# luigifreda/plvs

Hardware: AMD Instinct MI355X
Metric: Mvoxels/sec TSDF integrate (chisel 5 cm / 5 m, 640x480 RGB-D) (higher is better)
Workload: dtype f32; 1 GPU; configs[2] stand-in, STREAMING: see DESIGN.md 4.1 / 4.6; mode=order-free (fixed-point sums; sdf / weight within tolerance), longest_voxel_run=25008, parallelism=chunk-hash shard x1

## Files before the change

### plvs_amd/csrc/tsdf_walk.hpp

```cpp
#pragma once
#include <hip/hip_runtime.h>

#include <cstdint>

#include "tsdf_chisel_core.hpp"
#include "tsdf_directory.hpp"
#include "tsdf_tiles.hpp"
#include "tsdf_walk_table.hpp"

namespace {

using namespace plvs::chisel;
using plvs::tsdf::cloud_of;
using plvs::tsdf::tile_span;
using plvs::tsdf::tile_span_tables;
using plvs::tsdf::TileSpan;
using plvs::tsdf::kCoordBias;
using plvs::tsdf::kErrCoordRange;
using plvs::tsdf::kErrDirectoryMiss;
using plvs::tsdf::kErrPoolFull;
using plvs::tsdf::home_bucket;
using plvs::tsdf::next_bucket;

constexpr int kWalkRays = 512;
constexpr int kMaskWords = kWalkRays / 32;
#ifndef PLVS_WALK_ENTRIES
#define PLVS_WALK_ENTRIES 4096
#endif
constexpr int kWalkEntries = PLVS_WALK_ENTRIES;
constexpr int kWalkLimit = kWalkEntries * 7 / 8;
constexpr int kWalkWindow = kWalkLimit / 2;
constexpr int kWalkChunks = 64;
constexpr uint32_t kErrScratch = 8u;

#ifdef PLVS_WALK_PROF
__device__ unsigned long long g_walk_prof[16];
__device__ unsigned long long g_apply_items[8192][4];
#define WALK_PROF_BEGIN()                                         \
  long long prof_t = (long long)clock64();                        \
  unsigned long long prof_acc[9] = {0, 0, 0, 0, 0, 0, 0, 0, 0}
#define WALK_PROF(k)                                               \
  do {                                                             \
    const long long now = (long long)clock64();                    \
    prof_acc[k] += (unsigned long long)(now - prof_t);             \
    prof_t = now;                                                  \
  } while (0)
#define WALK_PROF_END()                                            \
  do {                                                             \
    if (threadIdx.x == 0)                                          \
      for (int k = 0; k < 9; ++k) atomicAdd(&g_walk_prof[k], prof_acc[k]); \
  } while (0)
#else
#define WALK_PROF_BEGIN() do {} while (0)
#define WALK_PROF(k) do {} while (0)
#define WALK_PROF_END() do {} while (0)
#endif

struct WalkCounters {
  unsigned long long total_visits;
  uint32_t err;
  uint32_t num_heads;
  uint32_t num_updated;
  uint32_t max_run;
  uint32_t num_desc;
  uint32_t run_need;
  uint32_t rec_top, seg_top;
  uint32_t ncold;
  uint32_t split_tiles;
  uint32_t num_parts;
  uint32_t num_multi;
  uint32_t ndeferred;
  uint32_t ndeferred2;
  uint32_t over_small;
  uint32_t skip;
  uint32_t collect_top;
  uint32_t collect_parts;
  uint32_t ndeferred3;
};

constexpr int kLogLen = 16;
constexpr int kSlabs = 8;
constexpr int kSlabVox = kChunkVox / kSlabs;

struct SubTile {
  uint16_t lo, hi;
  uint32_t vlo, vhi;
  int32_t cloud;
};

constexpr uint32_t kKeyEmpty = 0xFFFFFFFFu;
constexpr int kBuckets = kWalkEntries / 4;
constexpr int kOriginBias = 512;

constexpr int log2_of(int v) { return v <= 1 ? 0 : 1 + log2_of(v / 2); }
struct WalkShared {
  static constexpr int kEntries = kWalkEntries, kBucketCount = kWalkEntries / 4, kLogLen = ::kLogLen;
  alignas(16) uint32_t ekey[kWalkEntries];
  int32_t org[3];
  uint32_t cand[kWalkRays / 64];
  int32_t worg[kWalkRays / 64][3];
  uint32_t run_total, vis_total;
  uint32_t ccode[kWalkChunks];
  int32_t cslot[kWalkChunks];
  uint32_t ccnt[kWalkChunks * kSlabs];
  uint16_t cbase[kWalkChunks * kSlabs];
  uint32_t rbase;
  SubTile stack[16];
  int sp;
  uint32_t nent;
  uint32_t overflow;
  uint32_t wsum[kWalkRays / 64];
  uint32_t next, nrays;
};
template <int E>
struct FastShared {
  static constexpr int kEntries = E, kBucketCount = E / 4, kLogLen = E == 1536 ? ::kLogLen - 1 : ::kLogLen;
  static_assert(E % kWalkRays == 0 && E >= 1024, "every thread owns E / kWalkRays entries (and a bucket four)");
  alignas(16) uint32_t ekey[E];
  uint32_t cand[kWalkRays / 64];
  int32_t worg[kWalkRays / 64][3];
  uint32_t run_total, vis_total;
  uint32_t ccode[kWalkChunks];
  int32_t cslot[kWalkChunks];
  uint32_t ccnt[kWalkChunks * kSlabs];
  uint16_t cbase[kWalkChunks * kSlabs];
  uint32_t rcnt[kWalkChunks * kSlabs];
  uint16_t rcbase[kWalkChunks * kSlabs];
  uint32_t any_cold;
  uint32_t nent, overflow;
};


__device__ __forceinline__ bool rel_key(int vx, int vy, int vz, int ox, int oy, int oz, uint32_t* key) {
  const uint32_t dx = (uint32_t)(vx - ox), dy = (uint32_t)(vy - oy), dz = (uint32_t)(vz - oz);
  *key = dx | (dy << 10) | (dz << 20);
  return ((dx | dy | dz) >> 10) == 0u;
}
__device__ __forceinline__ int origin_of(int v) { return (v - kOriginBias) & ~15; }
constexpr uint32_t kChunkCodeMask = 0x3F0FC3F0u;
__device__ __forceinline__ uint32_t chunk_code(uint32_t key) { return key & kChunkCodeMask; }
__device__ __forceinline__ uint32_t voxel_in_chunk(uint32_t key) {
  return (key & 15u) | ((key >> 6) & 0xF0u) | ((key >> 12) & 0xF00u);
}
__device__ __forceinline__ void chunk_of_code(uint32_t code, int ox, int oy, int oz, int* cx, int* cy, int* cz) {
  *cx = (ox >> 4) + (int)((code >> 4) & 63u);
  *cy = (oy >> 4) + (int)((code >> 14) & 63u);
  *cz = (oz >> 4) + (int)((code >> 24) & 63u);
}
constexpr uint32_t kKeyMul = plvs::tsdf::kTableKeyMul, kKeyMulInv = plvs::tsdf::kTableKeyMulInv;
__device__ __forceinline__ uint32_t table_key(uint32_t key) { return key * kKeyMul; }
__device__ __forceinline__ uint32_t voxel_key(uint32_t tkey) { return tkey * kKeyMulInv; }
template <class SH>
__device__ __forceinline__ uint32_t key_bucket(uint32_t tkey) { return home_bucket<SH::kBucketCount>(tkey); }

__device__ __forceinline__ uint32_t wave_scan_incl(uint32_t x) {
  x += (uint32_t)__builtin_amdgcn_update_dpp(0, (int)x, 0x111, 0xf, 0xf, false);
  x += (uint32_t)__builtin_amdgcn_update_dpp(0, (int)x, 0x112, 0xf, 0xf, false);
  x += (uint32_t)__builtin_amdgcn_update_dpp(0, (int)x, 0x114, 0xf, 0xf, false);
  x += (uint32_t)__builtin_amdgcn_update_dpp(0, (int)x, 0x118, 0xf, 0xf, false);
  x += (uint32_t)__builtin_amdgcn_update_dpp(0, (int)x, 0x142, 0xa, 0xf, false);
// ... 669 lines not shown
      if (!own_region) {
        __syncthreads();
        rbase = S.rbase;
      }
#pragma unroll
      for (int k = 0; k < kPer; ++k) {
        if (slot_of[k] < 0) continue;
        const int e = tid + k * kWalkRays;
        const uint32_t vid = vkey[k] % (uint32_t)kChunkVox;
        const uint4 r = make_uint4(vid | ((uint32_t)(ewc[k] >> 32) << 12),
                                   grid ? grid_order_key(*grid, gt, elast[k]) : first + elast[k], (uint32_t)e_wuu[e],
                                   (uint32_t)ewc[k]);
        uint32_t at;
        if (ci[k] >= 0) {
          at = rbase + S.cbase[ci[k] * kSlabs + (int)(vid / kSlabVox)] + rank[k];
        } else {
          at = ntiles * rec_stride + atomicAdd(&ctr->rec_top, 1u);
          const uint32_t sg = ntiles * (uint32_t)kWalkChunks + atomicAdd(&ctr->seg_top, 1u);
          if (at >= out.rec_cap || sg >= out.seg_cap) {
            atomicOr(&ctr->err, kErrScratch);
          } else {
            uint32_t sub[kSlabs];
#pragma unroll
            for (int s = 0; s < kSlabs; ++s) sub[s] = (uint32_t)s > vid / kSlabVox ? 1u : 0u;
            out.seg[2 * (size_t)sg] = make_uint4((uint32_t)slot_of[k], at, 1u, gtile);
            out.seg[2 * (size_t)sg + 1] = pack_suboffsets(sub);
            if (out.chunk_nseg) atomicAdd(&out.chunk_nseg[slot_of[k]], 1u);
          }
        }
        if (at < out.rec_cap) out.rec[at] = r;
      }
    }

    ++flushes;
    WALK_PROF(6);
    if (!kRuns) {
      if (single && !was_split) break;
      continue;
    }
    uint32_t inc = nneed;
#pragma unroll
    for (int off = 1; off < 64; off <<= 1) {
      const uint32_t up = (uint32_t)__shfl_up((int)inc, off);
      if (lane >= off) inc += up;
    }
    const uint32_t wave_runs = (uint32_t)__shfl((int)inc, 63);
    if (!any_multi) {
      uint32_t base = 0;
      if (lane == 0 && wave_runs) base = atomicAdd(&S.run_total, wave_runs);
      base = (uint32_t)__shfl((int)base, 0);
      const bool fits_runs = base + wave_runs <= (1u << runs.r1_log2);
      if (!fits_runs && lane == 0) {
        atomicOr(&ctr->err, kErrScratch);
        atomicMax(&ctr->run_need, base + wave_runs);
      }
      uint32_t m = base + inc - nneed;
#pragma unroll
      for (int k = 0; k < kPer; ++k) {
        if (!(need & (1u << k)) || !fits_runs) continue;
        const size_t d = ((size_t)tile << runs.r1_log2) + m++;
        runs.dkey[d] = vkey[k];
        uint4* dst = reinterpret_cast<uint4*>(runs.masks + d * kMaskWords);
        const uint32_t word = elast[k] >> 5, bit = 1u << (elast[k] & 31u);
#pragma unroll
        for (int q = 0; q < kMaskWords / 4; ++q)
          dst[q] = make_uint4(word == 4u * q ? bit : 0u, word == 4u * q + 1u ? bit : 0u, word == 4u * q + 2u ? bit : 0u,
                              word == 4u * q + 3u ? bit : 0u);
      }
      WALK_PROF(7);
      if (single && !was_split) break;
      continue;
    }
    if (lane == 63) S.wsum[wid] = inc;
    __syncthreads();
    uint32_t wbase = 0, nruns = 0;
#pragma unroll
    for (int w = 0; w < kWalkRays / 64; ++w) {
      const uint32_t v = S.wsum[w];
      if (w < wid) wbase += v;
      nruns += v;
    }
    const uint32_t emitted = S.run_total;
    const bool fits_runs = emitted + nruns <= (1u << runs.r1_log2);
    if (!fits_runs && tid == 0) {
      atomicOr(&ctr->err, kErrScratch);
      atomicMax(&ctr->run_need, emitted + nruns);
    }
    {
      uint32_t m = wbase + inc - nneed;
#pragma unroll
      for (int k = 0; k < kPer; ++k) e_midx[tid + k * kWalkRays] = (need & (1u << k)) ? (uint16_t)m++ : (uint16_t)0xFFFFu;
    }
    for (uint32_t r0 = 0; fits_runs && r0 < nruns; r0 += kMaskCap) {
      __syncthreads();
#pragma unroll
      for (int k = 0; k < kMaskCap * kMaskWords / kWalkRays; ++k) raw[tid + k * kWalkRays] = 0u;
      __syncthreads();
      if (walks && nmine) {
        const uint32_t logged = min(nmine, (uint32_t)kLogLen);
        for (uint32_t k = 0; k < logged; ++k) {
          const uint32_t m = (uint32_t)e_midx[vlog[k * kWalkRays + tid]] - r0;
          if (m < (uint32_t)kMaskCap) atomicOr(&raw[m * kMaskWords + (tid >> 5)], 1u << (tid & 31));
        }
        if (nmine > (uint32_t)kLogLen) {
          walk_one(P, pose, ray, st.vlo, st.vhi, [&](uint32_t k, int vx, int vy, int vz, float) {
            if (k >= (uint32_t)kLogLen) {
              uint32_t key;
              const int e = rel_key(vx, vy, vz, fox, foy, foz, &key) ? table_find(S, table_key(key)) : -1;
              const uint32_t m = e >= 0 ? (uint32_t)e_midx[e] - r0 : 0xFFFFFFFFu;
              if (m < (uint32_t)kMaskCap) atomicOr(&raw[m * kMaskWords + (tid >> 5)], 1u << (tid & 31));
            }
            return true;
          });
        }
      }
      __syncthreads();
#pragma unroll
      for (int k = 0; k < kPer; ++k) {
        const uint32_t m = (uint32_t)e_midx[tid + k * kWalkRays];
        if (m == 0xFFFFu || m < r0 || m >= r0 + (uint32_t)kMaskCap) continue;
        const size_t d = ((size_t)tile << runs.r1_log2) + emitted + m;
        runs.dkey[d] = vkey[k];
        const uint32_t* mk = raw + (m - r0) * kMaskWords;
        uint4* dst = reinterpret_cast<uint4*>(runs.masks + d * kMaskWords);
#pragma unroll
        for (int q = 0; q < kMaskWords / 4; ++q) dst[q] = make_uint4(mk[4 * q], mk[4 * q + 1], mk[4 * q + 2], mk[4 * q + 3]);
      }
    }
    __syncthreads();
    if (tid == 0) S.run_total = emitted + nruns;
    WALK_PROF(7);
    if (single && !was_split) break;
  }

#pragma unroll
  for (int off = 32; off > 0; off >>= 1) my_visits += (uint32_t)__shfl_xor((int)my_visits, off);
  if (lane == 0 && my_visits) atomicAdd(&S.vis_total, my_visits);
  __syncthreads();
  if (tid == 0) {
    if (kRuns) runs.run_cnt[tile] = min(S.run_total, 1u << runs.r1_log2);
    if (kAcc) {
      out.tile_visits[tile] = S.vis_total;
      if (flushes == 0) out.seg_cnt[tile] = 0;
    }
    if (was_split) atomicAdd(&ctr->split_tiles, 1u);
  }
  WALK_PROF(8);
  WALK_PROF_END();
  }
}

constexpr int walk_fast_waves(int E) { return E > 2048 ? 2 : (E > 1536 ? 4 : 6); }
constexpr int kFastEntriesSmall = 1536;
template <int E, bool kGrid>
__device__ __forceinline__ void walk_fast_tile(
    const Params& P, float scale_u, float scale_w, const float* __restrict__ xyz, int npoints,
    const int32_t* __restrict__ offsets, int nclouds, const Pose* __restrict__ poses, const Directory& dir,
    int32_t* __restrict__ num_chunks, WalkCounters* __restrict__ ctr, const uint32_t* __restrict__ rgbw,
    const uint32_t* __restrict__ sat, const AccOut& out, const RunOut& runs, const TileMap& tmap, uint32_t rec_stride,
    uint32_t* __restrict__ deferred, uint32_t* __restrict__ ndeferred, const uint32_t tile, const bool listed_other,
    const GridSrc* __restrict__ grid_arg) {
  const GridSrc* __restrict__ const grid = kGrid ? grid_arg : nullptr;
  constexpr int kPer = E / kWalkRays;
  constexpr int kLimit = E * 7 / 8;
  constexpr int kMaskCapE = E / 4;
  constexpr int kLogLen = FastShared<E>::kLogLen;
  static_assert(kMaskCapE * kMaskWords % kWalkRays == 0, "the mask area is cleared by whole rounds of the tile's threads");
  __shared__ FastShared<E> S;
  __shared__ uint32_t raw[4 * E];
  __shared__ uint16_t vlog[kLogLen * kWalkRays];
  static_assert(offsetof(FastShared<E>, cbase) == offsetof(FastShared<E>, ccnt) + sizeof(S.ccnt), "cbase follows ccnt");
  constexpr bool kMidxOverlay = sizeof(S.ccnt) + sizeof(S.cbase) >= E * sizeof(uint16_t);
  __shared__ uint16_t e_midx_own[kMidxOverlay ? 1 : E];
  uint16_t* const e_midx = kMidxOverlay ? reinterpret_cast<uint16_t*>(S.ccnt) : e_midx_own;
  int32_t* const e_wuu = reinterpret_cast<int32_t*>(raw);
  unsigned long long* const e_wc = reinterpret_cast<unsigned long long*>(raw + E);
  uint32_t* const e_last = raw + 3 * E;
  const int tid = threadIdx.x, lane = tid & 63, wid = tid >> 6;
  const uint32_t gtile = tmap.tile_of(tile);
  const GridTile gt = grid ? grid_tile(*grid, gtile) : GridTile{0u, 0u, 0u};
  const TileSpan span = grid ? TileSpan{(int)gt.cloud, 0u, (uint32_t)kWalkRays}
                      : tmap.tables ? tile_span_tables(offsets, nclouds, gtile, kWalkRays)
                                    : tile_span(offsets, nclouds, gtile, kWalkRays);
  const uint32_t first = span.first, nrays = span.nrays;
  const int cloud = span.cloud;
  bool defer = P.shard_count > 1 || listed_other;
  WALK_PROF_BEGIN();
  uint32_t nv = 0;
  uint32_t rid = (uint32_t)threadIdx.x;
  bool walks = false;
  int ox = 0, oy = 0, oz = 0;
  if (!defer) {
    subtile_reset(S, tid);
#pragma unroll
    for (int k = 0; k < kWalkChunks * kSlabs / kWalkRays; ++k) S.rcnt[tid + k * kWalkRays] = 0u;
#pragma unroll
    for (int k = 0; k < 4 * kPer; ++k) raw[tid + k * kWalkRays] = 0u;
    if (tid == 0) {
      S.run_total = 0;
      S.vis_total = 0;
      S.any_cold = 0;
    }
    const Pose& pose = poses[cloud];
    Ray ray;
    walks = (uint32_t)tid < nrays && tile_ray_src(P, xyz, grid, gt, pose, first, rid, &ray, &ctr->err);
    const float wu = walks ? P.weight / (2.0f * ray.truncation) : 0.0f;
    {
      const unsigned long long wm = __ballot(walks);
      if (lane == 0) S.cand[wid] = wm ? 1u : 0u;
      if (wm && lane == __ffsll((long long)wm) - 1)
        for (int k = 0; k < 3; ++k) S.worg[wid][k] = origin_of((int)floorf(ray.start[k]));
    }
    WALK_PROF(0);
    __syncthreads();
    WALK_PROF(1);
    {
      int w0 = 0;
#pragma unroll
      for (int w = kWalkRays / 64 - 1; w >= 0; --w) w0 = S.cand[w] ? w : w0;
      ox = S.worg[w0][0]; oy = S.worg[w0][1]; oz = S.worg[w0][2];
      uint32_t anyc = 0;
#pragma unroll
      for (int w = 0; w < kWalkRays / 64; ++w) anyc |= S.cand[w];
      if (anyc == 0u) {
        if (tid == 0) {
          out.seg_cnt[tile] = 0;
          runs.run_cnt[tile] = 0;
          out.tile_visits[tile] = 0;
        }
        return;
      }
    }
    bool fits = false;
    if (walks) {
      const int reach = lean_reach(ray);
      const int rx = (int)floorf(ray.start[0]) - ox, ry = (int)floorf(ray.start[1]) - oy, rz = (int)floorf(ray.start[2]) - oz;
      fits = min(min(rx, ry), rz) - reach >= 0 && max(max(rx, ry), rz) + reach <= 1023;
      if (!fits) S.overflow = 1u;
    }
    if (fits) {
      nv = walk_lean<true, true>(P, pose, ray, S, ox, oy, oz, tid, wu * scale_u, (uint32_t)__float2int_rn(wu * scale_w), e_wuu,
                                 e_wc, e_last, vlog, rid);
    }
  }
  uint32_t ekey[kPer];
  WALK_PROF(2);
  if (!defer) {
    __syncthreads();
    WALK_PROF(3);
#pragma unroll
    for (int k = 0; k < kPer; ++k) {
      ekey[k] = S.ekey[tid + k * kWalkRays];
      if (ekey[k] != kKeyEmpty) ekey[k] = voxel_key(ekey[k]);
    }
    uint32_t wave_n = 0;
#pragma unroll
    for (int k = 0; k < kPer; ++k) wave_n += (uint32_t)__popcll(__ballot(ekey[k] != kKeyEmpty));
    if (lane == 0 && wave_n) atomicAdd(&S.nent, wave_n);
  } else {
#pragma unroll
    for (int k = 0; k < kPer; ++k) ekey[k] = kKeyEmpty;
  }
  int ci[kPer];
  uint32_t rank[kPer], rrank[kPer], vkey[kPer], elast[kPer];
  unsigned long long ewc[kPer];
  uint32_t need = 0;
  bool multi = false;
#pragma unroll
  for (int k = 0; k < kPer; ++k) {
    ci[k] = -2;
    rank[k] = 0;
    rrank[k] = 0;
    vkey[k] = 0xFFFFFFFFu;
    elast[k] = 0;
    ewc[k] = 0;
  }
  if (!defer) {
#pragma unroll
    for (int k = 0; k < kPer; ++k) {
      if (ekey[k] == kKeyEmpty) continue;
      bool won;
      ci[k] = chunk_cache_insert(S, chunk_code(ekey[k]), &won);
      if (ci[k] < 0) {
        S.overflow = 1u;
        continue;
      }
      int slot = S.cslot[ci[k]];
      if (slot < 0) {
        int cx, cy, cz;
        chunk_of_code(chunk_code(ekey[k]), ox, oy, oz, &cx, &cy, &cz);
        slot = dir_find_or_insert(dir, cx, cy, cz, num_chunks, &ctr->err);
        if (slot >= 0) S.cslot[ci[k]] = slot;
      }
      if (slot < 0) continue;
      vkey[k] = (uint32_t)slot * (uint32_t)kChunkVox + voxel_in_chunk(ekey[k]);
    }
    uint32_t cw[kPer];
#pragma unroll
    for (int k = 0; k < kPer; ++k) {
      cw[k] = 0u;
      if (vkey[k] != 0xFFFFFFFFu) cw[k] = sat ? sat[vkey[k] >> 5] : rgbw[vkey[k]];
    }
#pragma unroll
    for (int k = 0; k < kPer; ++k) {
      if (vkey[k] == 0xFFFFFFFFu) continue;
      const uint32_t vid = vkey[k] % (uint32_t)kChunkVox;
      ewc[k] = e_wc[tid + k * kWalkRays];
      elast[k] = e_last[tid + k * kWalkRays];
      rank[k] = atomicAdd(&S.ccnt[ci[k] * kSlabs + (int)(vid / kSlabVox)], 1u);
    }
#pragma unroll
    for (int k = 0; k < kPer; ++k) {
      if (vkey[k] == 0xFFFFFFFFu) continue;
      const bool cold = sat ? ((cw[k] >> (vkey[k] & 31u)) & 1u) == 0u : (cw[k] >> 24) < 254u;
      if (cold) {
        need |= 1u << k;
        multi = multi || (uint32_t)(ewc[k] >> 32) > 1u;
        rrank[k] = atomicAdd(&S.rcnt[ci[k] * kSlabs + (int)((vkey[k] % (uint32_t)kChunkVox) / kSlabVox)], 1u);
      }
    }
  }
  WALK_PROF(4);
  if (need) S.any_cold = 1u;
  const bool any_multi = __syncthreads_or(multi ? 1 : 0) != 0;
  const bool any_cold = S.any_cold != 0u;
  WALK_PROF(5);
  const bool too_many = !defer && S.nent > (uint32_t)kLimit;
  if (E == 2048 && tid == 0 && !defer && S.nent > (uint32_t)(kFastEntriesSmall * 7 / 8)) atomicAdd(&ctr->over_small, 1u);
  if (!defer) defer = S.overflow != 0 || too_many;
  if (defer) {
    if (tid == 0) {
      out.seg_cnt[tile] = 0;
      runs.run_cnt[tile] = 0;
      out.tile_visits[tile] = 0;
      deferred[atomicAdd(ndeferred, 1u)] = tile | (too_many ? 0x80000000u : 0u);
    }
    return;
  }
  {
    const uint32_t v = wave_sum(nv);
    if (lane == 0 && v) atomicAdd(&S.vis_total, v);
  }
  const uint32_t rbase = tile * rec_stride;
  uint32_t nruns;
  {
    uint32_t sub[kSlabs], c = 0, rsub[kSlabs], rc = 0;
#pragma unroll
    for (int s = 0; s < kSlabs; ++s) {
      sub[s] = c;
      c += S.ccnt[lane * kSlabs + s];
      rsub[s] = 0;
    }
    uint32_t rinc = 0;
    nruns = 0;
    if (any_cold) {
#pragma unroll
      for (int s = 0; s < kSlabs; ++s) {
        rsub[s] = rc;
        rc += S.rcnt[lane * kSlabs + s];
      }
      rinc = wave_scan_incl(rc);
      nruns = (uint32_t)__builtin_amdgcn_readlane((int)rinc, 63);
#pragma unroll
      for (int s = 0; s < kSlabs; ++s) S.rcbase[lane * kSlabs + s] = (uint16_t)(rinc - rc + rsub[s]);
    }
    const uint32_t both = wave_scan_incl(c | (c ? 1u << 16 : 0u));
    const uint32_t inc = both & 0xFFFFu, sinc = both >> 16;
#pragma unroll
    for (int s = 0; s < kSlabs; ++s) S.cbase[lane * kSlabs + s] = (uint16_t)(inc - c + sub[s]);
    if (wid == 0) {
      const uint32_t stot = (uint32_t)__builtin_amdgcn_readlane((int)sinc, 63);
      if (lane == 0) out.seg_cnt[tile] = stot;
      if (c) {
        const uint32_t sg = tile * (uint32_t)kWalkChunks + sinc - 1u;
        out.seg[2 * (size_t)sg] = make_uint4((uint32_t)S.cslot[lane], rbase + inc - c, c, gtile);
        out.seg[2 * (size_t)sg + 1] = pack_suboffsets(sub);
        if (runs.rseg) {
          runs.rseg[2 * (size_t)sg] = make_uint4((tile << runs.r1_log2) + rinc - rc, rc, 0u, 0u);
          runs.rseg[2 * (size_t)sg + 1] = pack_suboffsets(rsub);
        }
        if (out.chunk_nseg) atomicAdd(&out.chunk_nseg[S.cslot[lane]], 1u);
      }
    }
  }
#pragma unroll
  for (int k = 0; k < kPer; ++k) {
    if (vkey[k] == 0xFFFFFFFFu) continue;
    const uint32_t vid = vkey[k] % (uint32_t)kChunkVox;
    const uint4 r = make_uint4(vid | ((uint32_t)(ewc[k] >> 32) << 12),
                               grid ? grid_order_key(*grid, gt, elast[k]) : first + elast[k],
                               (uint32_t)e_wuu[tid + k * kWalkRays], (uint32_t)ewc[k]);
    out.rec[rbase + S.cbase[ci[k] * kSlabs + (int)(vid / kSlabVox)] + rank[k]] = r;
  }
  WALK_PROF(6);
  const bool fits_runs = nruns <= (1u << runs.r1_log2);
  if (!fits_runs && tid == 0) {
    atomicOr(&ctr->err, kErrScratch);
    atomicMax(&ctr->run_need, nruns);
  }
  uint32_t mrun[kPer];
#pragma unroll
  for (int k = 0; k < kPer; ++k)
    mrun[k] = (need & (1u << k)) ? (uint32_t)S.rcbase[ci[k] * kSlabs + (int)((vkey[k] % (uint32_t)kChunkVox) / kSlabVox)] + rrank[k] : 0xFFFFu;
  if (!any_multi) {
#pragma unroll
    for (int k = 0; k < kPer; ++k) {
      if (!(need & (1u << k)) || !fits_runs) continue;
      const size_t d = ((size_t)tile << runs.r1_log2) + mrun[k];
      runs.dkey[d] = vkey[k];
      uint4* dst = reinterpret_cast<uint4*>(runs.masks + d * kMaskWords);
      const uint32_t word = elast[k] >> 5, bit = 1u << (elast[k] & 31u);
#pragma unroll
      for (int q = 0; q < kMaskWords / 4; ++q)
        dst[q] = make_uint4(word == 4u * q ? bit : 0u, word == 4u * q + 1u ? bit : 0u, word == 4u * q + 2u ? bit : 0u,
                            word == 4u * q + 3u ? bit : 0u);
    }
  } else {
    __syncthreads();
#pragma unroll
    for (int k = 0; k < kPer; ++k) e_midx[tid + k * kWalkRays] = (uint16_t)mrun[k];
    for (uint32_t r0 = 0; fits_runs && r0 < nruns; r0 += kMaskCapE) {
      __syncthreads();
#pragma unroll
      for (int k = 0; k < kMaskCapE * kMaskWords / kWalkRays; ++k) raw[tid + k * kWalkRays] = 0u;
      __syncthreads();
      if (nv) {
        const uint32_t logged = min(nv, (uint32_t)kLogLen);
        for (uint32_t k = 0; k < logged; ++k) {
          const uint32_t m = (uint32_t)e_midx[vlog[k * kWalkRays + tid]] - r0;
          if (m < (uint32_t)kMaskCapE) atomicOr(&raw[m * kMaskWords + (rid >> 5)], 1u << (rid & 31));
        }
        if (nv > (uint32_t)kLogLen) {
          const Pose& pose = poses[cloud];
          Ray ray;
          if (tile_ray_src(P, xyz, grid, gt, pose, first, rid, &ray, &ctr->err))
            walk_one(P, pose, ray, 0u, 0xFFFFFFFFu, [&](uint32_t k, int vx, int vy, int vz, float) {
              if (k >= (uint32_t)kLogLen) {
                uint32_t key;
                const int e = rel_key(vx, vy, vz, ox, oy, oz, &key) ? table_find(S, table_key(key)) : -1;
                const uint32_t m = e >= 0 ? (uint32_t)e_midx[e] - r0 : 0xFFFFFFFFu;
                if (m < (uint32_t)kMaskCapE) atomicOr(&raw[m * kMaskWords + (rid >> 5)], 1u << (rid & 31));
              }
              return true;
            });
        }
      }
      __syncthreads();
#pragma unroll
      for (int k = 0; k < kPer; ++k) {
        const uint32_t m = (uint32_t)e_midx[tid + k * kWalkRays];
        if (m == 0xFFFFu || m < r0 || m >= r0 + (uint32_t)kMaskCapE) continue;
        const size_t d = ((size_t)tile << runs.r1_log2) + m;
        runs.dkey[d] = vkey[k];
        const uint32_t* mk = raw + (m - r0) * kMaskWords;
        uint4* dst = reinterpret_cast<uint4*>(runs.masks + d * kMaskWords);
#pragma unroll
        for (int q = 0; q < kMaskWords / 4; ++q) dst[q] = make_uint4(mk[4 * q], mk[4 * q + 1], mk[4 * q + 2], mk[4 * q + 3]);
      }
    }
  }
  if (tid == 0) S.run_total = nruns;
  WALK_PROF(7);
  __syncthreads();
  WALK_PROF(8);
  WALK_PROF_END();
  if (tid == 0) {
    runs.run_cnt[tile] = min(S.run_total, 1u << runs.r1_log2);
    out.tile_visits[tile] = S.vis_total;
  }
}

template <int E, bool kGrid = false>
__global__ __launch_bounds__(kWalkRays, walk_fast_waves(E)) void walk_fast(
    Params P, float scale_u, float scale_w, const float* __restrict__ xyz, int npoints,
    const int32_t* __restrict__ offsets, int nclouds, const Pose* __restrict__ poses, Directory dir,
    int32_t* __restrict__ num_chunks, WalkCounters* __restrict__ ctr, const uint32_t* __restrict__ rgbw,
    const uint32_t* __restrict__ sat, AccOut out, RunOut runs, TileMap tmap, uint32_t rec_stride,
    const uint32_t* __restrict__ tile_list, const uint32_t* __restrict__ ntile_list, uint32_t* __restrict__ deferred,
    uint32_t* __restrict__ ndeferred, const GridSrc* __restrict__ grid) {
  if (!tile_list) {
    walk_fast_tile<E, kGrid>(P, scale_u, scale_w, xyz, npoints, offsets, nclouds, poses, dir, num_chunks, ctr, rgbw, sat, out, runs,
                      tmap, rec_stride, deferred, ndeferred, blockIdx.x, false, grid);
    return;
  }
  const uint32_t nlist = *ntile_list;
  for (uint32_t lb = blockIdx.x; lb < nlist; lb += gridDim.x) {
    const uint32_t e = tile_list[lb];
    walk_fast_tile<E, kGrid>(P, scale_u, scale_w, xyz, npoints, offsets, nclouds, poses, dir, num_chunks, ctr, rgbw, sat, out, runs,
                      tmap, rec_stride, deferred, ndeferred, e & 0x7FFFFFFFu, (e >> 31) == 0u, grid);
    __syncthreads();
  }
}

constexpr int kSegSpan = 1024;
constexpr int kSegSpanLong = 4096;
constexpr uint32_t kPartSegs = 256;
constexpr uint32_t kPartMin = 512;
constexpr int kSegTable = 512;
template <bool kScatter, int kSpan = kSegSpan>
__global__ __launch_bounds__(256) void seg_pass(const uint4* __restrict__ seg, uint32_t seg_cap, uint32_t ntiles,
                                                const uint32_t* __restrict__ seg_cnt, uint32_t* __restrict__ chunk_nseg,
                                                const uint32_t* __restrict__ chunk_off, uint32_t* __restrict__ chunk_fill,
                                                uint4* __restrict__ sorted, const WalkCounters* __restrict__ ctr) {
  __shared__ uint32_t hkey[kSegTable], hcnt[kSegTable], hbase[kSegTable];
  const int tid = threadIdx.x;
  const uint32_t own = ntiles * (uint32_t)kWalkChunks;
  const uint32_t n = min(own + ctr->seg_top, seg_cap);
  for (int k = tid; k < kSegTable; k += 256) {
    hkey[k] = 0xFFFFFFFFu;
    hcnt[k] = 0;
  }
  __syncthreads();
  constexpr int kPer = kSpan / 256;
  int ent[kPer];
  uint32_t rnk[kPer], slot[kPer];
#pragma unroll
  for (int q = 0; q < kPer; ++q) {
    const uint32_t j = blockIdx.x * (uint32_t)kSpan + (uint32_t)(q * 256 + tid);
    ent[q] = -2;
    if (j >= n || (j < own && (j % kWalkChunks) >= seg_cnt[j / kWalkChunks])) continue;
    slot[q] = seg[2 * (size_t)j].x;
    uint32_t h = (slot[q] * 2654435761u) >> (32 - 9);
    ent[q] = -1;
    for (int probe = 0; probe < kSegTable; ++probe) {
      uint32_t cur = hkey[h];
      if (cur == 0xFFFFFFFFu) cur = atomicCAS(&hkey[h], 0xFFFFFFFFu, slot[q]);
      if (cur == 0xFFFFFFFFu || cur == slot[q]) {
        ent[q] = (int)h;
        break;
      }
      h = (h + 1) & (kSegTable - 1);
    }
    if (ent[q] >= 0) rnk[q] = atomicAdd(&hcnt[ent[q]], 1u);
  }
  __syncthreads();
  for (int k = tid; k < kSegTable; k += 256) {
    if (hkey[k] == 0xFFFFFFFFu) continue;
    if (kScatter) hbase[k] = chunk_off[hkey[k]] + atomicAdd(&chunk_fill[hkey[k]], hcnt[k]);
    else atomicAdd(&chunk_nseg[hkey[k]], hcnt[k]);
  }
  if (kScatter) __syncthreads();
#pragma unroll
  for (int q = 0; q < kPer; ++q) {
    if (ent[q] == -2) continue;
    const uint32_t j = blockIdx.x * (uint32_t)kSpan + (uint32_t)(q * 256 + tid);
    if (kScatter) {
      const uint32_t at = ent[q] >= 0 ? hbase[ent[q]] + rnk[q] : chunk_off[slot[q]] + atomicAdd(&chunk_fill[slot[q]], 1u);
      sorted[2 * (size_t)at] = seg[2 * (size_t)j];
      sorted[2 * (size_t)at + 1] = seg[2 * (size_t)j + 1];
    } else if (ent[q] == -1) {
      atomicAdd(&chunk_nseg[slot[q]], 1u);
    }
  }
}

__global__ __launch_bounds__(1024) void seg_scan(const uint32_t* __restrict__ chunk_nseg, uint32_t* __restrict__ chunk_off,
                                                 uint32_t* __restrict__ chunk_fill, uint32_t* __restrict__ active,
                                                 uint32_t* __restrict__ active_off, WalkCounters* __restrict__ ctr,
                                                 const int32_t* __restrict__ num_chunks, int max_chunks,
                                                 const uint32_t* __restrict__ tile_visits,
                                                 const uint32_t* __restrict__ run_cnt, uint32_t ntiles,
                                                 uint32_t* __restrict__ part_off, uint32_t* __restrict__ multi_idx,
                                                 uint32_t multi_cap, uint32_t part_segs, uint32_t part_min,
                                                 uint32_t* __restrict__ active_idx = nullptr) {
  __shared__ uint32_t wsum[16], wact[16], wprt[16], wmul[16];
  __shared__ uint32_t carry, acarry, pcarry, mcarry;
  __shared__ unsigned long long vsum[16];
  const int tid = threadIdx.x, lane = tid & 63, wid = tid >> 6;
  const int n = min(*num_chunks, max_chunks);
  if (tid == 0) { carry = 0; acarry = 0; pcarry = 0; mcarry = 0; }
  __syncthreads();
  for (int base = 0; base < n; base += 1024) {
    const int s = base + tid;
    const uint32_t c = s < n ? chunk_nseg[s] : 0u;
    const uint32_t a = c ? 1u : 0u;
    const uint32_t m = c > part_min ? 1u : 0u;
    uint32_t inc = c, ainc = a, minc = m;
#pragma unroll
    for (int off = 1; off < 64; off <<= 1) {
      const uint32_t up = (uint32_t)__shfl_up((int)inc, off), aup = (uint32_t)__shfl_up((int)ainc, off);
      const uint32_t mup = (uint32_t)__shfl_up((int)minc, off);
      if (lane >= off) { inc += up; ainc += aup; minc += mup; }
    }
    if (lane == 63) { wsum[wid] = inc; wact[wid] = ainc; wmul[wid] = minc; }
    __syncthreads();
    uint32_t wb = carry, ab = acarry, mb = mcarry, tot = 0, atot = 0, mtot = 0;
#pragma unroll
    for (int w = 0; w < 16; ++w) {
      if (w < wid) { wb += wsum[w]; ab += wact[w]; mb += wmul[w]; }
      tot += wsum[w];
      atot += wact[w];
      mtot += wmul[w];
    }
    const uint32_t midx = mb + minc - 1u;
    const bool multi = m && midx < multi_cap;
    const uint32_t np = multi ? (c + part_segs - 1u) / part_segs : a;
    uint32_t pinc = np;
#pragma unroll
    for (int off = 1; off < 64; off <<= 1) {
      const uint32_t pup = (uint32_t)__shfl_up((int)pinc, off);
      if (lane >= off) pinc += pup;
    }
    if (lane == 63) wprt[wid] = pinc;
    __syncthreads();
// ... 1353 lines not shown
```

Measured before the change: 85510 Mvoxels/s.

## Compact occupied hash entries into a dense list before per-entry processing

Occupied hash-table entries are first compacted into a dense index list using ballot and mbcnt prefix counts. Threads then process only live rounds, so whole rounds with no entries are skipped and lanes stay busy. Per-entry state (chunk index, rank, run index, last ray) is packed into two registers instead of several arrays, which should lower register pressure. The tile origin is made wave-uniform with readfirstlane. The cost is an extra barrier and scatter through e_last storage, which is reused as a list, and packed bitfields that depend on size limits checked by static_asserts.

```diff
diff --git a/plvs_amd/csrc/tsdf_walk.hpp b/plvs_amd/csrc/tsdf_walk.hpp
--- a/plvs_amd/csrc/tsdf_walk.hpp
+++ b/plvs_amd/csrc/tsdf_walk.hpp
@@ -6,6 +6,7 @@
 #include "tsdf_chisel_core.hpp"
 #include "tsdf_directory.hpp"
 #include "tsdf_tiles.hpp"
+#include "tsdf_walk_dense.hpp"
 #include "tsdf_walk_table.hpp"
 
 namespace {
@@ -981,6 +982,9 @@
 
 constexpr int walk_fast_waves(int E) { return E > 2048 ? 2 : (E > 1536 ? 4 : 6); }
 constexpr int kFastEntriesSmall = 1536;
+__device__ __forceinline__ int walk_group_of(uint32_t sa, uint32_t vkey) {
+  return (int)((sa >> 12) & 63u) * kSlabs + (int)((vkey % (uint32_t)kChunkVox) / (uint32_t)kSlabVox);
+}
 template <int E, bool kGrid>
 __device__ __forceinline__ void walk_fast_tile(
     const Params& P, float scale_u, float scale_w, const float* __restrict__ xyz, int npoints,
@@ -1047,7 +1051,9 @@
       int w0 = 0;
 #pragma unroll
       for (int w = kWalkRays / 64 - 1; w >= 0; --w) w0 = S.cand[w] ? w : w0;
-      ox = S.worg[w0][0]; oy = S.worg[w0][1]; oz = S.worg[w0][2];
+      ox = __builtin_amdgcn_readfirstlane(S.worg[w0][0]);
+      oy = __builtin_amdgcn_readfirstlane(S.worg[w0][1]);
+      oz = __builtin_amdgcn_readfirstlane(S.worg[w0][2]);
       uint32_t anyc = 0;
 #pragma unroll
       for (int w = 0; w < kWalkRays / 64; ++w) anyc |= S.cand[w];
@@ -1072,80 +1078,106 @@
                                  e_wc, e_last, vlog, rid);
     }
   }
-  uint32_t ekey[kPer];
+  uint32_t ekey[kPer], sa[kPer];
+  uint32_t nent = 0;
+#pragma unroll
+  for (int k = 0; k < kPer; ++k) {
+    ekey[k] = kKeyEmpty;
+    sa[k] = 0u;
+  }
   WALK_PROF(2);
   if (!defer) {
     __syncthreads();
     WALK_PROF(3);
+    uint16_t* const list = reinterpret_cast<uint16_t*>(e_last) + 1;
+    unsigned long long bal[kPer];
+    bool occ[kPer];
+    uint32_t wave_n = 0;
 #pragma unroll
     for (int k = 0; k < kPer; ++k) {
-      ekey[k] = S.ekey[tid + k * kWalkRays];
-      if (ekey[k] != kKeyEmpty) ekey[k] = voxel_key(ekey[k]);
-    }
-    uint32_t wave_n = 0;
-#pragma unroll
-    for (int k = 0; k < kPer; ++k) wave_n += (uint32_t)__popcll(__ballot(ekey[k] != kKeyEmpty));
-    if (lane == 0 && wave_n) atomicAdd(&S.nent, wave_n);
-  } else {
-#pragma unroll
-    for (int k = 0; k < kPer; ++k) ekey[k] = kKeyEmpty;
-  }
-  int ci[kPer];
-  uint32_t rank[kPer], rrank[kPer], vkey[kPer], elast[kPer];
-  unsigned long long ewc[kPer];
+      occ[k] = S.ekey[tid + k * kWalkRays] != kKeyEmpty;
+      bal[k] = __ballot(occ[k]);
+      wave_n += plvs::tsdf::dense_count(bal[k]);
+    }
+    if (wave_n) {
+      uint32_t base = 0;
+      if (lane == 0) base = atomicAdd(&S.nent, wave_n);
+      base = (uint32_t)__builtin_amdgcn_readfirstlane((int)base);
+      uint32_t earlier = 0;
+#pragma unroll
+      for (int k = 0; k < kPer; ++k) {
+        if (occ[k]) list[2u * plvs::tsdf::dense_index(base, earlier, bal[k], lane)] = (uint16_t)(tid + k * kWalkRays);
+        earlier += plvs::tsdf::dense_count(bal[k]);
+      }
+    }
+    __syncthreads();
+    nent = (uint32_t)__builtin_amdgcn_readfirstlane((int)S.nent);
+#pragma unroll
+    for (int k = 0; k < kPer; ++k) {
+      if (!plvs::tsdf::dense_round_live<kWalkRays>((uint32_t)k, nent)) break;
+      if (!plvs::tsdf::dense_owns<kWalkRays>((uint32_t)tid, (uint32_t)k, nent)) continue;
+      sa[k] = list[2u * plvs::tsdf::dense_place<kWalkRays>((uint32_t)tid, (uint32_t)k)];
+      ekey[k] = voxel_key(S.ekey[sa[k]]);
+    }
+  }
+  constexpr uint32_t kNoRun = 0xFFFu;
+  static_assert(E <= 4096 && kWalkChunks <= 64 && kSlabVox <= 4096 && kWalkRays <= 512, "the fields of sa and sb");
+  uint32_t vkey[kPer], sb[kPer];
   uint32_t need = 0;
   bool multi = false;
 #pragma unroll
   for (int k = 0; k < kPer; ++k) {
-    ci[k] = -2;
-    rank[k] = 0;
-    rrank[k] = 0;
     vkey[k] = 0xFFFFFFFFu;
-    elast[k] = 0;
-    ewc[k] = 0;
+    sb[k] = kNoRun;
   }
   if (!defer) {
 #pragma unroll
     for (int k = 0; k < kPer; ++k) {
+      if (!plvs::tsdf::dense_round_live<kWalkRays>((uint32_t)k, nent)) break;
       if (ekey[k] == kKeyEmpty) continue;
       bool won;
-      ci[k] = chunk_cache_insert(S, chunk_code(ekey[k]), &won);
-      if (ci[k] < 0) {
+      const int ci = chunk_cache_insert(S, chunk_code(ekey[k]), &won);
+      if (ci < 0) {
         S.overflow = 1u;
         continue;
       }
-      int slot = S.cslot[ci[k]];
+      sa[k] |= (uint32_t)ci << 12;
+      int slot = S.cslot[ci];
       if (slot < 0) {
         int cx, cy, cz;
         chunk_of_code(chunk_code(ekey[k]), ox, oy, oz, &cx, &cy, &cz);
         slot = dir_find_or_insert(dir, cx, cy, cz, num_chunks, &ctr->err);
-        if (slot >= 0) S.cslot[ci[k]] = slot;
+        if (slot >= 0) S.cslot[ci] = slot;
       }
       if (slot < 0) continue;
       vkey[k] = (uint32_t)slot * (uint32_t)kChunkVox + voxel_in_chunk(ekey[k]);
     }
-    uint32_t cw[kPer];
+    uint32_t cw[kPer], visits[kPer];
 #pragma unroll
     for (int k = 0; k < kPer; ++k) {
       cw[k] = 0u;
+      visits[k] = 0u;
+      if (!plvs::tsdf::dense_round_live<kWalkRays>((uint32_t)k, nent)) break;
       if (vkey[k] != 0xFFFFFFFFu) cw[k] = sat ? sat[vkey[k] >> 5] : rgbw[vkey[k]];
     }
 #pragma unroll
     for (int k = 0; k < kPer; ++k) {
+      if (!plvs::tsdf::dense_round_live<kWalkRays>((uint32_t)k, nent)) break;
       if (vkey[k] == 0xFFFFFFFFu) continue;
-      const uint32_t vid = vkey[k] % (uint32_t)kChunkVox;
-      ewc[k] = e_wc[tid + k * kWalkRays];
-      elast[k] = e_last[tid + k * kWalkRays];
-      rank[k] = atomicAdd(&S.ccnt[ci[k] * kSlabs + (int)(vid / kSlabVox)], 1u);
+      const uint32_t es = sa[k] & 0xFFFu;
+      visits[k] = (uint32_t)(e_wc[es] >> 32);
+      sb[k] |= (e_last[es] & 0xFFFFu) << 12;
+      sa[k] |= atomicAdd(&S.ccnt[walk_group_of(sa[k], vkey[k])], 1u) << 18;
     }
 #pragma unroll
     for (int k = 0; k < kPer; ++k) {
+      if (!plvs::tsdf::dense_round_live<kWalkRays>((uint32_t)k, nent)) break;
       if (vkey[k] == 0xFFFFFFFFu) continue;
       const bool cold = sat ? ((cw[k] >> (vkey[k] & 31u)) & 1u) == 0u : (cw[k] >> 24) < 254u;
       if (cold) {
         need |= 1u << k;
-        multi = multi || (uint32_t)(ewc[k] >> 32) > 1u;
-        rrank[k] = atomicAdd(&S.rcnt[ci[k] * kSlabs + (int)((vkey[k] % (uint32_t)kChunkVox) / kSlabVox)], 1u);
+        multi = multi || visits[k] > 1u;
+        sb[k] = (sb[k] & ~kNoRun) | atomicAdd(&S.rcnt[walk_group_of(sa[k], vkey[k])], 1u);
       }
     }
   }
@@ -1214,12 +1246,15 @@
   }
 #pragma unroll
   for (int k = 0; k < kPer; ++k) {
+    if (!plvs::tsdf::dense_round_live<kWalkRays>((uint32_t)k, nent)) break;
     if (vkey[k] == 0xFFFFFFFFu) continue;
     const uint32_t vid = vkey[k] % (uint32_t)kChunkVox;
-    const uint4 r = make_uint4(vid | ((uint32_t)(ewc[k] >> 32) << 12),
-                               grid ? grid_order_key(*grid, gt, elast[k]) : first + elast[k],
-                               (uint32_t)e_wuu[tid + k * kWalkRays], (uint32_t)ewc[k]);
-    out.rec[rbase + S.cbase[ci[k] * kSlabs + (int)(vid / kSlabVox)] + rank[k]] = r;
+    const uint32_t es = sa[k] & 0xFFFu, elast = sb[k] >> 12;
+    const unsigned long long ewc = e_wc[es];
+    const uint4 r = make_uint4(vid | ((uint32_t)(ewc >> 32) << 12),
+                               grid ? grid_order_key(*grid, gt, elast) : first + elast,
+                               (uint32_t)e_wuu[es], (uint32_t)ewc);
+    out.rec[rbase + S.cbase[walk_group_of(sa[k], vkey[k])] + (sa[k] >> 18)] = r;
   }
   WALK_PROF(6);
   const bool fits_runs = nruns <= (1u << runs.r1_log2);
@@ -1227,18 +1262,20 @@
     atomicOr(&ctr->err, kErrScratch);
     atomicMax(&ctr->run_need, nruns);
   }
-  uint32_t mrun[kPer];
-#pragma unroll
-  for (int k = 0; k < kPer; ++k)
-    mrun[k] = (need & (1u << k)) ? (uint32_t)S.rcbase[ci[k] * kSlabs + (int)((vkey[k] % (uint32_t)kChunkVox) / kSlabVox)] + rrank[k] : 0xFFFFu;
+#pragma unroll
+  for (int k = 0; k < kPer; ++k) {
+    if (!plvs::tsdf::dense_round_live<kWalkRays>((uint32_t)k, nent)) break;
+    if (need & (1u << k)) sb[k] += (uint32_t)S.rcbase[walk_group_of(sa[k], vkey[k])];
+  }
   if (!any_multi) {
 #pragma unroll
     for (int k = 0; k < kPer; ++k) {
+      if (!plvs::tsdf::dense_round_live<kWalkRays>((uint32_t)k, nent)) break;
       if (!(need & (1u << k)) || !fits_runs) continue;
-      const size_t d = ((size_t)tile << runs.r1_log2) + mrun[k];
+      const size_t d = ((size_t)tile << runs.r1_log2) + (sb[k] & kNoRun);
       runs.dkey[d] = vkey[k];
       uint4* dst = reinterpret_cast<uint4*>(runs.masks + d * kMaskWords);
-      const uint32_t word = elast[k] >> 5, bit = 1u << (elast[k] & 31u);
+      const uint32_t elast = sb[k] >> 12, word = elast >> 5, bit = 1u << (elast & 31u);
 #pragma unroll
       for (int q = 0; q < kMaskWords / 4; ++q)
         dst[q] = make_uint4(word == 4u * q ? bit : 0u, word == 4u * q + 1u ? bit : 0u, word == 4u * q + 2u ? bit : 0u,
@@ -1247,7 +1284,11 @@
   } else {
     __syncthreads();
 #pragma unroll
-    for (int k = 0; k < kPer; ++k) e_midx[tid + k * kWalkRays] = (uint16_t)mrun[k];
+    for (int k = 0; k < kPer; ++k) {
+      if (!plvs::tsdf::dense_round_live<kWalkRays>((uint32_t)k, nent)) break;
+      if (!plvs::tsdf::dense_owns<kWalkRays>((uint32_t)tid, (uint32_t)k, nent)) continue;
+      e_midx[sa[k] & 0xFFFu] = (need & (1u << k)) ? (uint16_t)(sb[k] & kNoRun) : (uint16_t)0xFFFFu;
+    }
     for (uint32_t r0 = 0; fits_runs && r0 < nruns; r0 += kMaskCapE) {
       __syncthreads();
 #pragma unroll
@@ -1277,8 +1318,9 @@
       __syncthreads();
 #pragma unroll
       for (int k = 0; k < kPer; ++k) {
-        const uint32_t m = (uint32_t)e_midx[tid + k * kWalkRays];
-        if (m == 0xFFFFu || m < r0 || m >= r0 + (uint32_t)kMaskCapE) continue;
+        if (!plvs::tsdf::dense_round_live<kWalkRays>((uint32_t)k, nent)) break;
+        const uint32_t m = sb[k] & kNoRun;
+        if (!(need & (1u << k)) || m < r0 || m >= r0 + (uint32_t)kMaskCapE) continue;
         const size_t d = ((size_t)tile << runs.r1_log2) + m;
         runs.dkey[d] = vkey[k];
         const uint32_t* mk = raw + (m - r0) * kMaskWords;
diff --git a/plvs_amd/csrc/tsdf_walk_dense.hpp b/plvs_amd/csrc/tsdf_walk_dense.hpp
--- /dev/null
+++ b/plvs_amd/csrc/tsdf_walk_dense.hpp
@@ -0,0 +1,48 @@
+#pragma once
+
+#include <cstdint>
+
+#if defined(__HIPCC__)
+#define PLVS_DENSE_FN __host__ __device__ __forceinline__
+#else
+#define PLVS_DENSE_FN inline
+#endif
+
+namespace plvs {
+namespace tsdf {
+
+constexpr int kDenseLanes = 64;
+
+PLVS_DENSE_FN uint32_t dense_below(uint64_t ballot, int lane) {
+#if defined(__HIP_DEVICE_COMPILE__)
+  (void)lane;
+  return __builtin_amdgcn_mbcnt_hi((uint32_t)(ballot >> 32), __builtin_amdgcn_mbcnt_lo((uint32_t)ballot, 0u));
+#else
+  return (uint32_t)__builtin_popcountll(ballot & ((1ull << lane) - 1ull));
+#endif
+}
+PLVS_DENSE_FN uint32_t dense_count(uint64_t ballot) { return (uint32_t)__builtin_popcountll(ballot); }
+
+PLVS_DENSE_FN uint32_t dense_index(uint32_t base, uint32_t earlier, uint64_t ballot, int lane) {
+  return base + earlier + dense_below(ballot, lane);
+}
+
+template <int kThreads>
+PLVS_DENSE_FN uint32_t dense_rounds(uint32_t nent) {
+  return (nent + (uint32_t)kThreads - 1u) / (uint32_t)kThreads;
+}
+template <int kThreads>
+PLVS_DENSE_FN bool dense_round_live(uint32_t k, uint32_t nent) {
+  return k * (uint32_t)kThreads < nent;
+}
+template <int kThreads>
+PLVS_DENSE_FN uint32_t dense_place(uint32_t tid, uint32_t k) {
+  return tid + k * (uint32_t)kThreads;
+}
+template <int kThreads>
+PLVS_DENSE_FN bool dense_owns(uint32_t tid, uint32_t k, uint32_t nent) {
+  return dense_place<kThreads>(tid, k) < nent;
+}
+
+}
+}
```

Measured after the change: 85410 Mvoxels/s. Within noise of the previous version (-0.1%).
